# Kitware/SMQTK-Indexing

Measured on AMD Instinct MI355X. Metric: queries/sec, exact brute-force l2 kNN k=100 over 10000000x128 float32 (recall@100 = 1.0 by construction); scan HBM GB/s vs 8 TB/s peak, higher is better.
Workload: dtype f32 results (distances bit-identical to numpy float32); filter arithmetic int8 MFMA (i32 accumulation, measured per-row error bound), exact re-rank f32

## Files before the change

### smqtk_indexing_amd/csrc/sq_common.hpp

```cpp
#pragma once
#include <hip/hip_runtime.h>

#include <atomic>
#include <chrono>

#include <cstdarg>
#include <cstdint>
#include <cstdio>
#include <cstring>
#include <mutex>
#include <string>
#include <unordered_map>
#include <utility>
#include <vector>

#include "../../include/smqtk_hip.h"

typedef unsigned long long u64;
typedef unsigned int u32;

namespace sq {

extern thread_local char g_err[512];
inline int fail(int code, const char* fmt, ...) {
// ... 34 lines not shown
    int dense_qplanes = 0;
    int dense_no_center = 0;
    int dense_rerank_segments = 0;
    int merge_threads = 0;
    int spin_wait_us = 2000;
    int dense_async_streams = 2;
    int dense_async_depth = 2;
    int dense_async_wait = 1;
    int dense_async_order = 1;
    int dense_nt = -1;
    int dense_nt_keep_mb = 0;
    int hamming_no_permute = 0;
    int dense_fused_prep = 1;
    int dense_int8_batch = 64;
    int dense_fused = 1;
    int dense_tighten = 1;
    int dense_graph = 1;
    int dense_int8 = -1;
    int dense_int8_wide = 0;
    int dense_mid_tier = 1;
    int hamming_async_depth = 2;
    int hamming_async_wait = 1;
    int hamming_async_order = 1;
    int hamming_ring = -1;
    int hamming_tighten = 1;
    int hamming_fused = 1;
};
extern Options g_opt;
int Options::*option_member(const char* name);

// ... 183 lines not shown
```

### smqtk_indexing_amd/csrc/sq_core.hip

```cpp
#include <algorithm>
#include <cmath>
#include <cstdint>
#include <cstring>
#include <limits>
#include <thread>
#include <utility>
#include <vector>

#include "sq_common.hpp"

namespace sq {

thread_local char g_err[512] = "";
Options g_opt;

static std::mutex g_reg_mu;
static std::unordered_map<sq_handle_t, HandleBase*> g_reg;
static sq_handle_t g_next = 1;

sq_handle_t register_handle(HandleBase* h) {
    std::lock_guard<std::mutex> l(g_reg_mu);
    sq_handle_t id = g_next++;
    g_reg[id] = h;
    return id;
// ... 53 lines not shown
        {"sample_stride", &Options::sample_stride},
        {"candidate_cap", &Options::candidate_cap},
        {"force_fallback", &Options::force_fallback},
        {"dense_stages", &Options::dense_stages},
        {"dense_blocks", &Options::dense_blocks},
        {"dense_sample_blocks", &Options::dense_sample_blocks},
        {"dense_debug", &Options::dense_debug},
        {"dense_waves", &Options::dense_waves},
        {"dense_qt", &Options::dense_qt},
        {"itq_exact", &Options::itq_exact},
        {"hamming_no_permute", &Options::hamming_no_permute},
        {"dense_no_center", &Options::dense_no_center},
        {"merge_threads", &Options::merge_threads},
        {"spin_wait_us", &Options::spin_wait_us},
        {"dense_rerank_segments", &Options::dense_rerank_segments},
        {"dense_qplanes", &Options::dense_qplanes},
        {"dense_async_streams", &Options::dense_async_streams},
        {"dense_async_depth", &Options::dense_async_depth},
        {"dense_async_wait", &Options::dense_async_wait},
        {"dense_async_order", &Options::dense_async_order},
        {"dense_nt", &Options::dense_nt},
        {"dense_nt_keep_mb", &Options::dense_nt_keep_mb},
        {"dense_mid_tier", &Options::dense_mid_tier},
        {"dense_int8", &Options::dense_int8},
        {"dense_int8_wide", &Options::dense_int8_wide},
        {"dense_graph", &Options::dense_graph},
        {"dense_fused", &Options::dense_fused},
        {"dense_tighten", &Options::dense_tighten},
        {"dense_int8_batch", &Options::dense_int8_batch},
        {"dense_fused_prep", &Options::dense_fused_prep},
// ... 311 lines not shown
```

### smqtk_indexing_amd/csrc/sq_dense.hip

```cpp
#include <algorithm>
#include <vector>
#include <cmath>

#include "sq_dense_exact.hpp"
#include "sq_dense_scan.hpp"
#include "sq_dense_mid.hpp"
#include "sq_dense_i8.hpp"
#include "sq_dense_wide.hpp"
#include "sq_dense_i8_wide.hpp"
#include "sq_dense_tighten.hpp"
#include "sq_dense_remove.hpp"

namespace sq {

struct DenseCall {
    bool pending = false;
    const float* q = nullptr;
    int nq = 0, k = 0, nq_pad = 0;
    void* out_dist = nullptr;
    long long* out_idx = nullptr;
    hipStream_t st = nullptr;
    bool small = false, all_fallback = false, prof = false, use_event = false, int8 = false;
    bool mid_direct = false;
    u32 cap = 0;
    sq_stats_t stats{};
};
struct DenseSlot {
    DevBuf q_scaled, q_al, qn2, thr, wave_out, wave_cnt, cnt, keys, sample, out_keys, cos_nq, oflag;
    DevBuf q8, par8;
    DevBuf clk8;
    int clk8_wgs = 0;
    DevBuf wave_score, hist8;
    DevBuf tg;
    void* tg_zeroed = nullptr;
    DevBuf sort_tmp;
    HostPinned status_host;
    HostPinned call_ptrs;
// ... 252 lines not shown
template <int KS>
static int dense8_head_launch_t(const Dense8HeadArgs& a, hipStream_t st) {
    using G = I8Geom<KS>;
    constexpr int ring = G::WAVES * G::NSTAGE * G::SLOT_BYTES;
    return launch_lds<dense8_head_kernel<KS>>(ring, dim3((unsigned)a.s.nrb), dim3(G::WAVES * 64), ring, st, a);
}
static int dense8_head_launch(int row_bytes, const Dense8HeadArgs& a, hipStream_t st) {
    switch (row_bytes) {
        case 128: return dense8_head_launch_t<4>(a, st);
        case 256: return dense8_head_launch_t<8>(a, st);
        case 512: return dense8_head_launch_t<16>(a, st);
    }
    return fail(SQ_ERR_INVALID, "int8 head: unsupported row width %d", row_bytes);
}
template <int KS, bool COSINE>
static int dense8_body_launch_t(const Dense8ScanArgs& a, const Dense8TailArgs& t, hipStream_t st) {
    using G = I8Geom<KS>;
    constexpr int ring = G::WAVES * G::NSTAGE * G::SLOT_BYTES;
    return launch_lds<dense8_body_kernel<KS, COSINE>>(ring, dim3((unsigned)a.nrb), dim3(G::WAVES * 64), ring, st, a, t);
}
static int dense8_body_launch(int row_bytes, bool cosine, const Dense8ScanArgs& a, const Dense8TailArgs& t, hipStream_t st) {
    switch (row_bytes) {
        case 128: return cosine ? dense8_body_launch_t<4, true>(a, t, st) : dense8_body_launch_t<4, false>(a, t, st);
        case 256: return cosine ? dense8_body_launch_t<8, true>(a, t, st) : dense8_body_launch_t<8, false>(a, t, st);
        case 512: return cosine ? dense8_body_launch_t<16, true>(a, t, st) : dense8_body_launch_t<16, false>(a, t, st);
    }
    return fail(SQ_ERR_INVALID, "int8 body: unsupported row width %d", row_bytes);
}
static int i8_waves(int row_bytes) { return row_bytes == 512 ? I8Geom<16>::WAVES : I8Geom<4>::WAVES; }

static bool dense_mid_shape_ok(const DenseHandle* h) {
    const bool cosine = h->metric == SQ_METRIC_COSINE;
    return h->d <= 512 && (reinterpret_cast<uintptr_t>(h->db) & 15u) == 0 && (h->ld & 3) == 0 && h->ld >= (h->d + 3) / 4 * 4 && h->n >= 32 &&
           (cosine ? h->cos_nx.p != nullptr : h->norms.p != nullptr);
}

static int dense8_wide_enqueue(DenseHandle* h, DenseSlot& s, const float* q, int nq, int k, int kk, void* out_dist, long long* out_idx,
                               hipStream_t st, bool prof, u32 cap, u32* hs_dev, u32* hs_raw_dev) {
    const long long n = h->n;
    const int d = h->d, row8 = h->row8, ku = i8w_units(row8), qw = ku * I8W_UNIT;
    const bool cosine = h->metric == SQ_METRIC_COSINE;
    const size_t key_bytes = cosine ? sizeof(K128) : sizeof(u64);
// ... 310 lines not shown
            else if (per_wg <= 4.5 && keep8 > 8) keep8 = 8;
        }
        const long long lane_m = (long long)nrb_sample * keep8;
        SQ_TRY(s.sample.reserve(fused ? (size_t)TILE_ROWS * lane_m * 4 : (size_t)nq_pad * ns * 4));
        a.sample_out = s.sample.as<float>();
        if (fused) {
            SQ_TRY(s.wave_score.reserve((size_t)n_waves * wave_cap * 4));
            SQ_TRY(s.hist8.reserve((size_t)I8_HIST_WORDS * 4));
            a.wave_score = s.wave_score.as<float>();
            a.hist = s.hist8.as<u32>();
        }
        int wpb = 2;
        if (!cosine && h->opt.dense_rerank_segments > 0 && waves8 % h->opt.dense_rerank_segments == 0 && h->opt.dense_rerank_segments <= 4)
            wpb = h->opt.dense_rerank_segments;
        const size_t rr_lds = (qt == 1 && ldq <= 156) ? (size_t)32 * (ldq + 4) * 4 : 0;
        const DenseCallPtrs* ind = nullptr;
        auto chain = [&](hipStream_t cs) -> int {
            if (fused) {
                Dense8HeadArgs ha{};
                ha.s = a;
                ha.s.unit_step = stride;
                ha.s.n_sel = ns_units;
                ha.s.nrb = nrb_sample;
                ha.q = q;
                ha.nq = nq;
                ha.d = d;
                ha.center = centerp;
                ha.dx = h->dx8;
                ha.r_max = h->rmax8;
                ha.x_max = h->xmax8;
                ha.cosine = cosine ? 1 : 0;
                ha.qn2 = qn2;
                ha.cnt = cnt;
                ha.oflag = oflag;
                ha.q_al = s.q_al.as<float>();
                ha.ldq = ldq;
                ha.ind = ind;
                ha.lane_min = s.sample.as<float>();
                ha.keep = keep8;
                ha.kk = kk;
                if (const int rc = dense8_head_launch(row8, ha, cs)) return rc;
                Dense8ScanArgs b = a;
                b.unit_step = 1;
                b.n_sel = n_units;
                b.nrb = nrb;
                Dense8TailArgs ta{h->db, h->ld, d, s.q_al.as<float>(), ldq, nq, s.keys.p, cnt, cap, oflag, cnx, cnq, h->opt.dense_debug, qn2, kk, tighten ? 1 : 0, nullptr};
                s.clk8_wgs = 0;
                if ((h->opt.dense_debug & 8192) && !use_event) {
                    if (const int rc = s.clk8.reserve((size_t)nrb * 64)) return rc;
                    SQ_HIP(hipMemsetAsync(s.clk8.p, 0, (size_t)nrb * 64, cs));
                    ta.clk = s.clk8.as<long long>();
                    s.clk8_wgs = nrb;
                }
                if (prof) SQ_HIP(hipEventRecord(s.ev[1], cs));
                if (const int rc = dense8_body_launch(row8, cosine, b, ta, cs)) return rc;
                if (prof) {
                    SQ_HIP(hipEventRecord(s.ev[2], cs));
                    SQ_HIP(hipEventRecord(s.ev[4], cs));
                }
                if (cosine) {
                    DenseFinalizeCos fin{cnt, cap, kk, h->id_base, thr, 0.0, 1, (double*)out_dist, out_idx, hs_dev, hs_raw_dev, oflag, 0};
                    fin.lin = s.par8.as<float2>();
                    fin.ind = ind;
                    if (tighten) fin.thr2k = a.hist + TILE_ROWS * I8_HIST_BINS;
                    fin.cnt_shift = I8_CNT_SHIFT;
                    return select_launch_t<K128>(s.keys.as<K128>(), cnt, cap, key_stride, k, nq, s.out_keys.as<K128>(), fin, cs, s.sort_tmp, 8 * stride * kk, I8_CNT_SHIFT);
                }
                DenseFinalizeL2 fin{cnt, cap, kk, h->id_base, thr, qn2, 0.0, 1, (float*)out_dist, out_idx, hs_dev, hs_raw_dev, oflag, 0};
                fin.lin = s.par8.as<float2>();
                fin.ind = ind;
                if (tighten) fin.thr2k = a.hist + TILE_ROWS * I8_HIST_BINS;
                fin.cnt_shift = I8_CNT_SHIFT;
                return select_launch_t<u64>(s.keys.as<u64>(), cnt, cap, key_stride, k, nq, s.out_keys.as<u64>(), fin, cs, s.sort_tmp, 8 * stride * kk, I8_CNT_SHIFT);
            }
// ... 24 lines not shown
                fin.lin = s.par8.as<float2>();
                fin.ind = ind;
                return select_launch_t<K128>(s.keys.as<K128>(), cnt, cap, key_stride, k, nq, s.out_keys.as<K128>(), fin, cs, s.sort_tmp, 8 * stride * kk);
            }
            hipLaunchKernelGGL(dense_rerank_l2_kernel, dim3((unsigned)((n_waves + wpb - 1) / wpb)), dim3(128 * wpb), rr_lds, cs, h->db, h->ld, d,
                               s.q_al.as<float>(), ldq, a.wave_out, a.wave_cnt, wave_cap, n_waves, wpb, nq, group_q, s.keys.as<u64>(), cnt,
                               cap, oflag, h->opt.dense_debug);
            if (prof) SQ_HIP(hipEventRecord(s.ev[4], cs));
            DenseFinalizeL2 fin{cnt, cap, kk, h->id_base, thr, qn2, 0.0, 1, (float*)out_dist, out_idx, hs_dev, hs_raw_dev, oflag, 0};
            fin.lin = s.par8.as<float2>();
            fin.ind = ind;
            return select_launch_t<u64>(s.keys.as<u64>(), cnt, cap, key_stride, k, nq, s.out_keys.as<u64>(), fin, cs, s.sort_tmp, 8 * stride * kk);
        };
        c.stats.scan_launches = 2;
        c.stats.bytes_scanned = h->n_pad64 * ((long long)row8 + 4) * nqt;
        bool launched = false;
        if (use_event && !prof && h->opt.dense_graph != 0 && !h->graph_broken && st != nullptr && st == s.own) {
            u64 key = 0xcbf29ce484222325ull;
            auto mix = [&key](u64 v) { key = (key ^ v) * 0x100000001b3ull; };
            for (u64 v : {(u64)(fused ? 1 : 0), (u64)(tighten ? 1 : 0), (u64)(uintptr_t)s.wave_score.p, (u64)(uintptr_t)s.hist8.p, (u64)lane_m, (u64)nq, (u64)k, (u64)row8, (u64)qt, (u64)nqt, (u64)wpb, (u64)stride, (u64)nrb, (u64)nrb_sample, (u64)ns, (u64)a.nt, (u64)a.nt_from_row, (u64)n, (u64)h->n_live, (u64)cap,
                          (u64)h->opt.dense_debug, (u64)h->id_base, (u64)(uintptr_t)st, (u64)(uintptr_t)h->db, (u64)(uintptr_t)centerp,
                          (u64)(uintptr_t)h->scan8.p, (u64)(uintptr_t)h->nrow8.p, (u64)(uintptr_t)s.q8.p, (u64)(uintptr_t)s.par8.p,
                          (u64)(uintptr_t)s.sample.p, (u64)(uintptr_t)s.keys.p, (u64)(uintptr_t)s.wave_out.p, (u64)(uintptr_t)s.wave_cnt.p,
                          (u64)(uintptr_t)s.q_al.p, (u64)(uintptr_t)cnt, (u64)(uintptr_t)thr, (u64)(uintptr_t)qn2, (u64)(uintptr_t)oflag,
                          (u64)(uintptr_t)s.out_keys.p, (u64)(uintptr_t)hs_raw_dev, (u64)(uintptr_t)cnx, (u64)(uintptr_t)cnq, (u64)(cosine ? 1 : 0)})
                mix(v);
            if (key == 0) key = 1;
            if (s.gexec && s.gkey != key) {
                (void)hipGraphExecDestroy(s.gexec);
                s.gexec = nullptr;
            }
            if (!s.gexec && s.seen_key == key) {
                SQ_TRY(s.call_ptrs.reserve(sizeof(DenseCallPtrs)));
                void* ind_dev = nullptr;
                SQ_TRY(s.call_ptrs.device_ptr(&ind_dev));
// ... 223 lines not shown
    u32* cnt = s.cnt.as<u32>();
    float* thr = s.thr.as<float>();
    double* qn2 = s.qn2.as<double>();
    const double* cnx = h->cos_nx.as<double>();
    const double* cnq = s.cos_nq.as<double>();
    u32* hs_raw = reinterpret_cast<u32*>(s.status_host.p);
    u32* hs = hs_raw + c.nq_pad;
    u32* hs_raw_dev = nullptr;
    SQ_TRY(s.status_host.device_ptr(reinterpret_cast<void**>(&hs_raw_dev)));
    u32* hs_dev = hs_raw_dev + c.nq_pad;
    const size_t l2_lds = (size_t)((d + 3) / 4 * 4) * 4;
    h->stats = c.stats;
    if (!all_fallback) {
        SQ_HIP(c.use_event ? event_wait(s.ev_done) : stream_wait(st));
        SQ_HIP(hipGetLastError());
        double clk_tail_ms = -1.0;
        if (s.clk8_wgs > 0 && (h->opt.dense_debug & 8192)) {
            std::vector<long long> ck((size_t)s.clk8_wgs * 8);
            SQ_HIP(hipMemcpy(ck.data(), s.clk8.p, ck.size() * 8, hipMemcpyDeviceToHost));
            long long t0 = ck[0], tend = 0;
            for (int w = 0; w < s.clk8_wgs; ++w) t0 = std::min(t0, ck[(size_t)w * 8]), tend = std::max(tend, ck[(size_t)w * 8 + 4]);
            double sum[5] = {0, 0, 0, 0, 0}, mx[5] = {0, 0, 0, 0, 0}, mn[5] = {1e30, 1e30, 1e30, 1e30, 1e30};
            for (int w = 0; w < s.clk8_wgs; ++w) {
                const long long* e = &ck[(size_t)w * 8];
                const double v[5] = {(e[0] - t0) * 0.01, (e[1] - e[0]) * 0.01, (e[2] - e[1]) * 0.01, (e[3] - e[2]) * 0.01, (e[4] - e[3]) * 0.01};
                for (int j = 0; j < 5; ++j) sum[j] += v[j], mx[j] = std::max(mx[j], v[j]), mn[j] = std::min(mn[j], v[j]);
            }
            const char* names[5] = {"start offset", "stream (first wave out)", "wave skew (all waves out)", "thresholds", "re-rank"};
            if (h->opt.dense_debug & 16384) {
                fprintf(stderr, "[body clocks] %d workgroups, kernel span %.1f us\n", s.clk8_wgs, (tend - t0) * 0.01);
                for (int j = 0; j < 5; ++j) fprintf(stderr, "   %-28s min %8.1f  mean %8.1f  max %8.1f us\n", names[j], mn[j], sum[j] / s.clk8_wgs, mx[j]);
            }
            long long stream_end = 0;
            for (int w = 0; w < s.clk8_wgs; ++w) stream_end = std::max(stream_end, ck[(size_t)w * 8 + 2]);
            clk_tail_ms = (double)(tend - stream_end) * 1e-5;
            s.clk8_wgs = 0;
        }
        if (c.prof) {
            float t1 = 0, t2 = 0;
            SQ_HIP(hipEventElapsedTime(&t1, s.ev[1], s.ev[2]));
            SQ_HIP(hipEventElapsedTime(&t2, s.ev[0], s.ev[3]));
            h->stats.scan_ms = t1;
            h->stats.total_ms = t2;
            if (h->ev_ref) {
                float e[5] = {0, 0, 0, 0, 0};
                const int order[5] = {0, 1, 2, 4, 3};
                for (int j = 0; j < 5; ++j) (void)hipEventElapsedTime(&e[j], h->ev_ref, s.ev[order[j]]);
                fprintf(stderr, "[smqtk_hip] trace slot %d: start %.1f | head-> %.1f | scan-> %.1f | rerank-> %.1f | select-> %.1f us\n",
                        (int)(&s - h->slot), e[0] * 1e3f, e[1] * 1e3f, e[2] * 1e3f, e[3] * 1e3f, e[4] * 1e3f);
            }
            if (c.stats.scan_launches == 2) {
                float t3 = 0;
                SQ_HIP(hipEventElapsedTime(&t3, s.ev[2], s.ev[4]));
                h->stats.rerank_ms = t3;
                if (clk_tail_ms >= 0.0) h->stats.rerank_ms = clk_tail_ms;
            }
        }
        for (int qi = 0; qi < nq; ++qi) h->stats.candidates += hs_raw[qi];
        if (c.int8) {
            int over = 0;
            for (int qi = 0; qi < nq; ++qi) over += (hs[qi] & 1u) ? 1 : 0;
            long long cands = 0;
            for (int qi = 0; qi < nq; ++qi) cands += hs_raw[qi];
            const bool heavy = 2 * over > nq || cands > (long long)nq * std::max<long long>(24ll * 1024, n / 128);
            h->overflow8 = heavy ? h->overflow8 + 1 : 0;
            if (h->overflow8 >= 3 && h->opt.dense_int8 < 0) h->suspended8 = true;
        }
        if (!small && (!c.int8 || h->opt.dense_int8 > 0)) {
            int over = 0;
            for (int qi = 0; qi < nq; ++qi) over += (hs[qi] & 1u) ? 1 : 0;
// ... 1090 lines not shown
```

### smqtk_indexing_amd/csrc/sq_dense_i8.hpp

```cpp
#pragma once
#include "sq_dense_scan.hpp"

namespace sq {

typedef int i32x4 __attribute__((ext_vector_type(4)));
typedef int i32x16 __attribute__((ext_vector_type(16)));

template <int KS>
struct I8Geom {
    static constexpr int ROW_BYTES = KS * 32;
    static constexpr int UNIT_ROWS = KS == 4 ? 64 : 32;
    static constexpr int TILES = UNIT_ROWS / 32;
    static constexpr int UNIT_BYTES = UNIT_ROWS * ROW_BYTES;
    static constexpr int SLOT_BYTES = UNIT_BYTES + 256;
    static constexpr int WAVES = KS <= 8 ? 8 : 4;
    static constexpr int NSTAGE = 2;
    static constexpr int PIECES = UNIT_BYTES / 1024;
    static constexpr int SAMPLES_PER_UNIT = 2 * TILES;
};
static constexpr int I8_MAX_ROW_BYTES = 512;
__host__ __device__ constexpr int i8_row_bytes(int d) { return d <= 128 ? 128 : (d <= 256 ? 256 : 512); }
__host__ __device__ constexpr int i8_unit_rows(int row_bytes) { return row_bytes == 128 ? 64 : 32; }

__device__ __forceinline__ float i8_element(float v, const float* __restrict__ center, int k, bool cosine, double inv_norm) {
// ... 364 lines not shown
};

template <int KS>
__device__ __forceinline__ int i8_swz(int c, int r) {
    if constexpr (KS == 4) return c ^ ((r >> 1) & 7);
    return (c & ~15) | ((c & 15) ^ (r & 15));
}

enum { I8_EMIT = 0, I8_SAMPLE = 1, I8_LANEMIN = 2, I8_EMIT_H = 3 };

static constexpr int I8_HIST_BINS = 64;
static constexpr int I8_CNT_SHIFT = 5;
static constexpr int I8_HIST_WORDS = TILE_ROWS * I8_HIST_BINS + (TILE_ROWS << I8_CNT_SHIFT);

template <int WAVES>
__device__ __forceinline__ void dense8_hist_flush(u32* lds_hist, u32* __restrict__ ghist) {
    constexpr int PER = TILE_ROWS * I8_HIST_BINS / WAVES;
    const int lane = threadIdx.x & 63;
    const int wave = __builtin_amdgcn_readfirstlane(threadIdx.x >> 6);
#pragma unroll
    for (int i = 0; i < PER / 64; ++i) {
        const int b = wave * PER + i * 64 + lane;
        const u32 v = __hip_atomic_exchange(lds_hist + b, 0u, __ATOMIC_RELAXED, __HIP_MEMORY_SCOPE_WORKGROUP);
        if (v) __hip_atomic_fetch_add(ghist + b, v, __ATOMIC_RELAXED, __HIP_MEMORY_SCOPE_AGENT);
    }
}

template <int KS, int MODE>
__device__ __forceinline__ void dense8_stream(const Dense8ScanArgs& a, unsigned char* smem, const i32x4 (&bq)[KS], const i32x4 (&bl)[KS],
                                              float unit_lo, float thr_l, u32& wcount, float& smin, u32* lds_ticket,
                                              float inv_w_l = 0.f, u32* lds_hist = nullptr) {
    using G = I8Geom<KS>;
    constexpr bool SAMPLE = MODE == I8_SAMPLE || MODE == I8_LANEMIN;
    const int lane = threadIdx.x & 63;
    const int wave = __builtin_amdgcn_readfirstlane(threadIdx.x >> 6);
    const int r31 = lane & 31, h = lane >> 5;
    const u32 lds_base = (u32)(uintptr_t)smem;
    const u32 ring_base = lds_base + (u32)wave * (G::NSTAGE * G::SLOT_BYTES);
    const unsigned char* ring_ptr = smem + wave * (G::NSTAGE * G::SLOT_BYTES);
    const long long wave_id = (long long)blockIdx.x * G::WAVES + wave;
    const long long nwaves = (long long)a.nrb * G::WAVES;
    uint2* wout = a.wave_out + wave_id * a.wave_cap;
    float* wsc = MODE == I8_EMIT_H ? a.wave_score + wave_id * a.wave_cap : nullptr;
    u32* hist_l = MODE == I8_EMIT_H ? lds_hist + r31 * I8_HIST_BINS : nullptr;

    const long long wg_first = (long long)blockIdx.x * G::WAVES;
    auto take_unit = [&]() __attribute__((always_inline)) -> long long {
        u32 t = 0;
        if (lane == 0) t = __hip_atomic_fetch_add(lds_ticket, 1u, __ATOMIC_RELAXED, __HIP_MEMORY_SCOPE_WORKGROUP);
        t = (u32)__builtin_amdgcn_readfirstlane((int)t);
        const long long u = wg_first + (long long)(t % G::WAVES) + (long long)(t / G::WAVES) * nwaves;
        return u < a.n_sel ? u : -1ll;
    };
    const long long my_units = wave_id < a.n_sel ? (a.n_sel - wave_id + nwaves - 1) / nwaves : 0;
    u32 voff[G::PIECES];
#pragma unroll
    for (int j = 0; j < G::PIECES; ++j) {
        const int lin = j * 1024 + lane * 16;
        const int r = lin / G::ROW_BYTES, cpos = (lin % G::ROW_BYTES) >> 4;
        voff[j] = (u32)(r * G::ROW_BYTES + i8_swz<KS>(cpos, r) * 16);
    }
    const u32 voff_n = (u32)lane * 4u;
    static_assert(G::NSTAGE == 2, "two ring slots: the units in flight are sel_even / sel_odd");
    long long issued = 0, sel_even = -1, sel_odd = -1;
    bool more = true;
    auto issue_next = [&]() __attribute__((always_inline)) {
        if (!more) return;
        const long long sel = take_unit();
        if (sel < 0) {
// ... 4 lines not shown
        const long long unit_idx = sel * a.unit_step;
        const long long row0 = unit_idx * G::UNIT_ROWS;
        const u32 dst = ring_base + (u32)(issued % G::NSTAGE) * G::SLOT_BYTES;
        const unsigned char* base = reinterpret_cast<const unsigned char*>(a.scan8) + row0 * G::ROW_BYTES;
#pragma unroll
        for (int j = 0; j < G::PIECES; ++j) {
            if (a.nt && row0 >= a.nt_from_row)
                glds16<true>(base, voff[j], dst + (u32)j * 1024);
            else
                glds16<false>(base, voff[j], dst + (u32)j * 1024);
        }
        glds4(a.nrow + row0, voff_n, dst + G::UNIT_BYTES);
        ++issued;
    };
    for (int p = 0; p < G::NSTAGE; ++p) issue_next();
    const int flush_every = (int)(my_units >> 3) > 0 ? (int)(my_units >> 3) : 1;
    int to_flush = flush_every;

    for (long long it = 0; it < issued; ++it) {
        const long long sel = (it & 1) ? sel_odd : sel_even;
        const long long unit_idx = sel * a.unit_step;
        const long long row0 = unit_idx * G::UNIT_ROWS;
        wait_units_in_flight<G::NSTAGE, G::PIECES + 1>((int)(issued - it - 1));
        const unsigned char* sl = ring_ptr + (it % G::NSTAGE) * G::SLOT_BYTES;
        constexpr int KH = KS == 16 ? 8 : KS;
        i32x4 av[G::TILES][KH];
        f32x4 nr[G::TILES][4];
#pragma unroll
        for (int t = 0; t < G::TILES; ++t) {
            const int r = 32 * t + r31;
#pragma unroll
            for (int s = 0; s < KH; ++s)
                av[t][s] = *reinterpret_cast<const i32x4*>(sl + r * G::ROW_BYTES + i8_swz<KS>(2 * s + h, r) * 16);
// ... 52 lines not shown
                    if (mask) {
                        const u32 pos = wcount + __builtin_amdgcn_mbcnt_hi((u32)(bal >> 32), __builtin_amdgcn_mbcnt_lo((u32)bal, 0u));
                        if (pos < a.wave_cap) {
                            wout[pos] = make_uint2((u32)(row0 + 32 * t + 4 * h), (mask << 16) | (u32)r31);
                            if constexpr (MODE == I8_EMIT_H) wsc[pos] = m;
                        }
                        if constexpr (MODE == I8_EMIT_H) {
                            if (m > -__builtin_inff()) {
                                const int bin = min((int)((thr_l - m) * inv_w_l), I8_HIST_BINS - 1);
                                __hip_atomic_fetch_add(hist_l + bin, 1u, __ATOMIC_RELAXED, __HIP_MEMORY_SCOPE_WORKGROUP);
                            }
                        }
                    }
                    wcount += (u32)__popcll(bal);
                }
            }
        }
        if constexpr (MODE == I8_EMIT_H) {
            if (--to_flush == 0) {
                to_flush = flush_every;
                dense8_hist_flush<G::WAVES>(lds_hist, a.hist);
            }
        }
    }
}

template <int KS>
__device__ __forceinline__ void dense8_load_planes(const signed char* planes, i32x4 (&bq)[KS], i32x4 (&bl)[KS]) {
    using G = I8Geom<KS>;
    const int lane = threadIdx.x & 63, r31 = lane & 31, h = lane >> 5;
#pragma unroll
    for (int s = 0; s < KS; ++s) {
        bq[s] = *reinterpret_cast<const i32x4*>(planes + r31 * G::ROW_BYTES + (2 * s + h) * 16);
        bl[s] = *reinterpret_cast<const i32x4*>(planes + (TILE_ROWS + r31) * G::ROW_BYTES + (2 * s + h) * 16);
    }
#pragma unroll
// ... 223 lines not shown
    const float* db;
    long long ld;
    int d;
    const float* q_al;
    int ldq, nq;
    void* keys;
    u32* cnt;
    u32 cap;
    u32* overflow;
    const double* nx64;
    const double* nq64;
    int debug;
    const double* qn2;
    int kk;
    int tighten;
    long long* clk;
};
static constexpr int I8_TAIL_QROWS_BYTES = 32 * (156 + 4) * 4;
static constexpr int I8_TAIL_LIST = 2048;
static constexpr int I8_TAIL_RERANK_BYTES = I8_TAIL_QROWS_BYTES + 3 * RERANK_MAX_GROUP * 4 + 8 * 32 * RERANK_STAGE_STRIDE * 4;
static constexpr int I8_TAIL_LDS_BYTES = I8_TAIL_RERANK_BYTES + I8_TAIL_LIST * 8 + TILE_ROWS * 4 + 16;

template <int KS, bool COSINE>
__global__ __launch_bounds__(I8Geom<KS>::WAVES * 64, KS == 16 ? 1 : 2) void dense8_body_kernel(Dense8ScanArgs a, Dense8TailArgs ta) {
    using G = I8Geom<KS>;
    static_assert(I8_TAIL_LDS_BYTES <= G::WAVES * G::NSTAGE * G::SLOT_BYTES, "the re-rank works in the ring's LDS");
    extern __shared__ __attribute__((aligned(16))) unsigned char smem[];
    __shared__ u32 s_hist8[TILE_ROWS * I8_HIST_BINS];
    __shared__ u32 s_wcnt[G::WAVES];
    __shared__ u32 s_unit_ticket;
    __shared__ float s_thr1[TILE_ROWS], s_eq[TILE_ROWS];
    __shared__ double s_qn2b[TILE_ROWS];
    __shared__ float2 s_parb[TILE_ROWS];
    if (threadIdx.x == 0) s_unit_ticket = 0u;
    if (threadIdx.x < TILE_ROWS) {
        s_thr1[threadIdx.x] = a.thr[threadIdx.x];
        s_parb[threadIdx.x] = a.par[threadIdx.x];
        s_eq[threadIdx.x] = a.par[threadIdx.x].y;
        s_qn2b[threadIdx.x] = ta.qn2[threadIdx.x];
    }
    const int lane = threadIdx.x & 63;
    const int wave = __builtin_amdgcn_readfirstlane(threadIdx.x >> 6);
    const int r31 = lane & 31;
    for (int i = threadIdx.x; i < TILE_ROWS * I8_HIST_BINS; i += G::WAVES * 64) s_hist8[i] = 0u;
    long long* clk = ta.clk ? ta.clk + (long long)blockIdx.x * 8 : nullptr;
    if (clk && threadIdx.x == 0) {
        clk[0] = (long long)wall_clock64();
        clk[1] = 0x7fffffffffffffffll;
    }
    __syncthreads();
    i32x4 bq[KS], bl[KS];
    dense8_load_planes<KS>(a.qs8, bq, bl);
    float unit_lo = a.par[r31].x * 0.00390625f;
    float thr_l = a.thr[r31];
    const float eq_l = a.par[r31].y;
    float inv_w_l = (eq_l > 0.f && eq_l < __builtin_inff()) ? 2.f / eq_l : 0.f;
    if (!(inv_w_l < 3.0e38f)) inv_w_l = 0.f;
    asm volatile("" : "+v"(unit_lo), "+v"(thr_l), "+v"(inv_w_l));
    u32 wcount = 0;
    float smin = 0.f;
    dense8_stream<KS, I8_EMIT_H>(a, smem, bq, bl, unit_lo, thr_l, wcount, smin, &s_unit_ticket, inv_w_l, s_hist8);
    const long long w0 = (long long)blockIdx.x * G::WAVES;
    if (lane == 0) {
        a.wave_cnt[2 * (w0 + wave)] = wcount;
        a.wave_cnt[2 * (w0 + wave) + 1] = 0u;
        s_wcnt[wave] = wcount;
        if (clk) atomicMin((unsigned long long*)(clk + 1), (unsigned long long)wall_clock64());
    }
    asm volatile("s_waitcnt vmcnt(0) lgkmcnt(0)" ::: "memory");
    __builtin_amdgcn_fence(__ATOMIC_RELEASE, "workgroup");
    __syncthreads();
    __builtin_amdgcn_fence(__ATOMIC_ACQUIRE, "workgroup");
    if (clk && threadIdx.x == 0) clk[2] = (long long)wall_clock64();
    float* fl = reinterpret_cast<float*>(smem);
    u32* su = reinterpret_cast<u32*>(smem + I8_TAIL_QROWS_BYTES);
    RerankLds L{fl, su, su + RERANK_MAX_GROUP, su + 2 * RERANK_MAX_GROUP,
                COSINE ? reinterpret_cast<float*>(smem + I8_TAIL_QROWS_BYTES + 3 * RERANK_MAX_GROUP * 4) : nullptr};
    {
        uint2* s_list = reinterpret_cast<uint2*>(smem + I8_TAIL_RERANK_BYTES);
        float* s_thr2 = reinterpret_cast<float*>(smem + I8_TAIL_RERANK_BYTES + I8_TAIL_LIST * 8);
        u32* s_npass = reinterpret_cast<u32*>(s_thr2 + TILE_ROWS);
        static_assert(I8_HIST_BINS == 64, "one lane per bin");
        bool any = false;
#pragma unroll
        for (int wi = 0; wi < G::WAVES; ++wi) any = any || s_wcnt[wi] != 0u;
        const Dense8ThrPost post{s_parb, s_qn2b};
        constexpr int NQW = TILE_ROWS / G::WAVES;
        u32 hc[NQW];
        if (ta.tighten && any) {
#pragma unroll
            for (int j = 0; j < NQW; ++j) {
                const int qi = (j >> 2) * 4 * G::WAVES + wave * 4 + (j & 3);
                hc[j] = __hip_atomic_load(a.hist + qi * I8_HIST_BINS + lane, __ATOMIC_RELAXED, __HIP_MEMORY_SCOPE_AGENT);
            }
#pragma unroll
            for (int j = 0; j < NQW; ++j) {
                const int qi = (j >> 2) * 4 * G::WAVES + wave * 4 + (j & 3);
                hc[j] += s_hist8[qi * I8_HIST_BINS + lane];
            }
        }
#pragma unroll
        for (int rnd = 0; rnd < TILE_ROWS / (4 * G::WAVES); ++rnd) {
#pragma unroll
            for (int j = 0; j < 4; ++j) {
                const int qi = rnd * 4 * G::WAVES + wave * 4 + j;
                const float t1 = s_thr1[qi];
                float t2 = t1;
                if (ta.tighten && any && qi < ta.nq && t1 < __builtin_inff() && t1 > -__builtin_inff()) {
                    u32 c = hc[rnd * 4 + j];
#pragma unroll
                    for (int o = 1; o < 64; o <<= 1) {
                        const u32 up = (u32)__shfl_down((int)c, o);
                        c += lane + o < 64 ? up : 0u;
                    }
                    const u64 reach = __ballot(c >= (u32)ta.kk);
                    const float eq = s_eq[qi];
                    if (reach != 0ull && eq > 0.f && eq < __builtin_inff()) {
                        const int jb = 63 - __clzll((long long)reach);
                        const float inv_w = 2.f / eq;
                        if (inv_w < 3.0e38f) {
                            const double t8 = (double)t1 - (double)jb / (double)inv_w * (1.0 - 1e-6);
                            float t8f = (float)t8;
                            if ((double)t8f < t8) t8f = __uint_as_float(__float_as_uint(t8f) + (t8f >= 0.f ? 1 : -1));
                            const float cand = post(qi, t8f);
                            if (cand < t2) t2 = cand;
                        }
                    }
                    if (lane == 0) atomicMax(a.hist + TILE_ROWS * I8_HIST_BINS + (qi << I8_CNT_SHIFT), ordered_f32(t2));
                }
                if (lane == 0) s_thr2[qi] = t2;
            }
        }
        if (ta.tighten) {
            L.scores = a.wave_score;
            L.thr2 = s_thr2;
            L.list = s_list;
            L.npass = s_npass;
            L.list_cap = I8_TAIL_LIST;
        }
        L.seg_cnt = s_wcnt;
        L.cnt_shift = I8_CNT_SHIFT;
        __syncthreads();
        if (clk && threadIdx.x == 0) clk[3] = (long long)wall_clock64();
        if (ta.tighten) dense8_hist_flush<G::WAVES>(s_hist8, a.hist);
    }
    using K = typename std::conditional<COSINE, K128, u64>::type;
    rerank_block<K, COSINE>(ta.db, ta.ld, ta.d, ta.q_al, ta.ldq, ta.nq, TILE_ROWS, a.wave_out, a.wave_cnt, a.wave_cap,
                            (long long)a.nrb * G::WAVES, G::WAVES, static_cast<K*>(ta.keys), ta.cnt, ta.cap, ta.overflow, ta.nx64,
                            ta.nq64, ta.debug, w0, L);
    if (clk) {
        asm volatile("s_waitcnt vmcnt(0) lgkmcnt(0)" ::: "memory");
        __syncthreads();
        if (threadIdx.x == 0) clk[4] = (long long)wall_clock64();
    }
}

template <int QT, bool SAMPLE>
__global__ __launch_bounds__(512, 2) void dense8_scan_mt_kernel(Dense8ScanArgs a) {
    using G = I8Geom<4>;
    extern __shared__ __attribute__((aligned(16))) unsigned char smem[];
    const int lane = threadIdx.x & 63;
    const int wave = __builtin_amdgcn_readfirstlane(threadIdx.x >> 6);
    const int r31 = lane & 31, h = lane >> 5;
    const u32 lds_base = (u32)(uintptr_t)smem;
    const u32 ring_base = lds_base + (u32)wave * (G::NSTAGE * G::SLOT_BYTES);
    const unsigned char* ring_ptr = smem + wave * (G::NSTAGE * G::SLOT_BYTES);
    const long long wave_id = (long long)blockIdx.x * G::WAVES + wave;
    uint2* wout = a.wave_out + wave_id * a.wave_cap;
// ... 124 lines not shown
```

Before: 144,000.

## Split fused int8 body kernel into separate scan and tail re-rank kernels

```diff
diff --git a/smqtk_indexing_amd/csrc/sq_common.hpp b/smqtk_indexing_amd/csrc/sq_common.hpp
--- a/smqtk_indexing_amd/csrc/sq_common.hpp
+++ b/smqtk_indexing_amd/csrc/sq_common.hpp
@@ -72,6 +72,7 @@
     int dense_fused_prep = 1;
     int dense_int8_batch = 64;
     int dense_fused = 1;
+    int dense_tail_blocks = 0;
     int dense_tighten = 1;
     int dense_graph = 1;
     int dense_int8 = -1;
diff --git a/smqtk_indexing_amd/csrc/sq_core.hip b/smqtk_indexing_amd/csrc/sq_core.hip
--- a/smqtk_indexing_amd/csrc/sq_core.hip
+++ b/smqtk_indexing_amd/csrc/sq_core.hip
@@ -91,6 +91,7 @@
         {"merge_threads", &Options::merge_threads},
         {"spin_wait_us", &Options::spin_wait_us},
         {"dense_rerank_segments", &Options::dense_rerank_segments},
+        {"dense_tail_blocks", &Options::dense_tail_blocks},
         {"dense_qplanes", &Options::dense_qplanes},
         {"dense_async_streams", &Options::dense_async_streams},
         {"dense_async_depth", &Options::dense_async_depth},
diff --git a/smqtk_indexing_amd/csrc/sq_dense.hip b/smqtk_indexing_amd/csrc/sq_dense.hip
--- a/smqtk_indexing_amd/csrc/sq_dense.hip
+++ b/smqtk_indexing_amd/csrc/sq_dense.hip
@@ -21,6 +21,7 @@
     long long* out_idx = nullptr;
     hipStream_t st = nullptr;
     bool small = false, all_fallback = false, prof = false, use_event = false, int8 = false;
+    bool tail_in_scan = false;
     bool mid_direct = false;
     u32 cap = 0;
     sq_stats_t stats{};
@@ -303,18 +304,22 @@
     return fail(SQ_ERR_INVALID, "int8 head: unsupported row width %d", row_bytes);
 }
 template <int KS, bool COSINE>
-static int dense8_body_launch_t(const Dense8ScanArgs& a, const Dense8TailArgs& t, hipStream_t st) {
+static int dense8_body_launch_t(const Dense8ScanArgs& a, long long* clk, hipStream_t st) {
     using G = I8Geom<KS>;
     constexpr int ring = G::WAVES * G::NSTAGE * G::SLOT_BYTES;
-    return launch_lds<dense8_body_kernel<KS, COSINE>>(ring, dim3((unsigned)a.nrb), dim3(G::WAVES * 64), ring, st, a, t);
-}
-static int dense8_body_launch(int row_bytes, bool cosine, const Dense8ScanArgs& a, const Dense8TailArgs& t, hipStream_t st) {
+    return launch_lds<dense8_body_kernel<KS, COSINE>>(ring, dim3((unsigned)a.nrb), dim3(G::WAVES * 64), ring, st, a, clk);
+}
+static int dense8_body_launch(int row_bytes, bool cosine, const Dense8ScanArgs& a, long long* clk, hipStream_t st) {
     switch (row_bytes) {
-        case 128: return cosine ? dense8_body_launch_t<4, true>(a, t, st) : dense8_body_launch_t<4, false>(a, t, st);
-        case 256: return cosine ? dense8_body_launch_t<8, true>(a, t, st) : dense8_body_launch_t<8, false>(a, t, st);
-        case 512: return cosine ? dense8_body_launch_t<16, true>(a, t, st) : dense8_body_launch_t<16, false>(a, t, st);
+        case 128: return cosine ? dense8_body_launch_t<4, true>(a, clk, st) : dense8_body_launch_t<4, false>(a, clk, st);
+        case 256: return cosine ? dense8_body_launch_t<8, true>(a, clk, st) : dense8_body_launch_t<8, false>(a, clk, st);
+        case 512: return cosine ? dense8_body_launch_t<16, true>(a, clk, st) : dense8_body_launch_t<16, false>(a, clk, st);
     }
     return fail(SQ_ERR_INVALID, "int8 body: unsupported row width %d", row_bytes);
+}
+static int dense8_tail_launch(bool cosine, int blocks, size_t lds, const Dense8TailArgs& t, hipStream_t st) {
+    return cosine ? launch<dense8_tail_kernel<true>>(dim3((unsigned)blocks), dim3(I8_TAIL_WAVES * 64), lds, st, t)
+                  : launch<dense8_tail_kernel<false>>(dim3((unsigned)blocks), dim3(I8_TAIL_WAVES * 64), lds, st, t);
 }
 static int i8_waves(int row_bytes) { return row_bytes == 512 ? I8Geom<16>::WAVES : I8Geom<4>::WAVES; }
 
@@ -655,6 +660,7 @@
         if (!cosine && h->opt.dense_rerank_segments > 0 && waves8 % h->opt.dense_rerank_segments == 0 && h->opt.dense_rerank_segments <= 4)
             wpb = h->opt.dense_rerank_segments;
         const size_t rr_lds = (qt == 1 && ldq <= 156) ? (size_t)32 * (ldq + 4) * 4 : 0;
+        const int tail_blocks = h->opt.dense_tail_blocks > 0 ? h->opt.dense_tail_blocks : nrb;
         const DenseCallPtrs* ind = nullptr;
         auto chain = [&](hipStream_t cs) -> int {
             if (fused) {
@@ -685,20 +691,45 @@
                 b.unit_step = 1;
                 b.n_sel = n_units;
                 b.nrb = nrb;
-                Dense8TailArgs ta{h->db, h->ld, d, s.q_al.as<float>(), ldq, nq, s.keys.p, cnt, cap, oflag, cnx, cnq, h->opt.dense_debug, qn2, kk, tighten ? 1 : 0, nullptr};
+                long long* clk = nullptr;
                 s.clk8_wgs = 0;
                 if ((h->opt.dense_debug & 8192) && !use_event) {
                     if (const int rc = s.clk8.reserve((size_t)nrb * 64)) return rc;
                     SQ_HIP(hipMemsetAsync(s.clk8.p, 0, (size_t)nrb * 64, cs));
-                    ta.clk = s.clk8.as<long long>();
+                    clk = s.clk8.as<long long>();
                     s.clk8_wgs = nrb;
                 }
                 if (prof) SQ_HIP(hipEventRecord(s.ev[1], cs));
-                if (const int rc = dense8_body_launch(row8, cosine, b, ta, cs)) return rc;
-                if (prof) {
-                    SQ_HIP(hipEventRecord(s.ev[2], cs));
-                    SQ_HIP(hipEventRecord(s.ev[4], cs));
-                }
+                if (const int rc = dense8_body_launch(row8, cosine, b, clk, cs)) return rc;
+                if (prof) SQ_HIP(hipEventRecord(s.ev[2], cs));
+                Dense8TailArgs ta{};
+                ta.db = h->db;
+                ta.ld = h->ld;
+                ta.d = d;
+                ta.q_al = s.q_al.as<float>();
+                ta.ldq = ldq;
+                ta.nq = nq;
+                ta.keys = s.keys.p;
+                ta.cnt = cnt;
+                ta.cap = cap;
+                ta.overflow = oflag;
+                ta.nx64 = cnx;
+                ta.nq64 = cnq;
+                ta.debug = h->opt.dense_debug;
+                ta.qn2 = qn2;
+                ta.kk = kk;
+                ta.tighten = tighten ? 1 : 0;
+                ta.par = a.par;
+                ta.thr = thr;
+                ta.wave_out = a.wave_out;
+                ta.wave_score = a.wave_score;
+                ta.wave_cnt = a.wave_cnt;
+                ta.wave_cap = wave_cap;
+                ta.n_waves = n_waves;
+                ta.segs = waves8;
+                ta.hist = a.hist;
+                if (const int rc = dense8_tail_launch(cosine, std::min(tail_blocks, nrb), rr_lds, ta, cs)) return rc;
+                if (prof) SQ_HIP(hipEventRecord(s.ev[4], cs));
                 if (cosine) {
                     DenseFinalizeCos fin{cnt, cap, kk, h->id_base, thr, 0.0, 1, (double*)out_dist, out_idx, hs_dev, hs_raw_dev, oflag, 0};
                     fin.lin = s.par8.as<float2>();
@@ -753,11 +784,12 @@
         };
         c.stats.scan_launches = 2;
         c.stats.bytes_scanned = h->n_pad64 * ((long long)row8 + 4) * nqt;
+        c.tail_in_scan = fused;
         bool launched = false;
         if (use_event && !prof && h->opt.dense_graph != 0 && !h->graph_broken && st != nullptr && st == s.own) {
             u64 key = 0xcbf29ce484222325ull;
             auto mix = [&key](u64 v) { key = (key ^ v) * 0x100000001b3ull; };
-            for (u64 v : {(u64)(fused ? 1 : 0), (u64)(tighten ? 1 : 0), (u64)(uintptr_t)s.wave_score.p, (u64)(uintptr_t)s.hist8.p, (u64)lane_m, (u64)nq, (u64)k, (u64)row8, (u64)qt, (u64)nqt, (u64)wpb, (u64)stride, (u64)nrb, (u64)nrb_sample, (u64)ns, (u64)a.nt, (u64)a.nt_from_row, (u64)n, (u64)h->n_live, (u64)cap,
+            for (u64 v : {(u64)(fused ? 1 : 0), (u64)(tighten ? 1 : 0), (u64)tail_blocks, (u64)(uintptr_t)s.wave_score.p, (u64)(uintptr_t)s.hist8.p, (u64)lane_m, (u64)nq, (u64)k, (u64)row8, (u64)qt, (u64)nqt, (u64)wpb, (u64)stride, (u64)nrb, (u64)nrb_sample, (u64)ns, (u64)a.nt, (u64)a.nt_from_row, (u64)n, (u64)h->n_live, (u64)cap,
                           (u64)h->opt.dense_debug, (u64)h->id_base, (u64)(uintptr_t)st, (u64)(uintptr_t)h->db, (u64)(uintptr_t)centerp,
                           (u64)(uintptr_t)h->scan8.p, (u64)(uintptr_t)h->nrow8.p, (u64)(uintptr_t)s.q8.p, (u64)(uintptr_t)s.par8.p,
                           (u64)(uintptr_t)s.sample.p, (u64)(uintptr_t)s.keys.p, (u64)(uintptr_t)s.wave_out.p, (u64)(uintptr_t)s.wave_cnt.p,
@@ -1011,31 +1043,27 @@
     if (!all_fallback) {
         SQ_HIP(c.use_event ? event_wait(s.ev_done) : stream_wait(st));
         SQ_HIP(hipGetLastError());
-        double clk_tail_ms = -1.0;
         if (s.clk8_wgs > 0 && (h->opt.dense_debug & 8192)) {
             std::vector<long long> ck((size_t)s.clk8_wgs * 8);
             SQ_HIP(hipMemcpy(ck.data(), s.clk8.p, ck.size() * 8, hipMemcpyDeviceToHost));
             long long t0 = ck[0], tend = 0;
-            for (int w = 0; w < s.clk8_wgs; ++w) t0 = std::min(t0, ck[(size_t)w * 8]), tend = std::max(tend, ck[(size_t)w * 8 + 4]);
-            double sum[5] = {0, 0, 0, 0, 0}, mx[5] = {0, 0, 0, 0, 0}, mn[5] = {1e30, 1e30, 1e30, 1e30, 1e30};
+            for (int w = 0; w < s.clk8_wgs; ++w) t0 = std::min(t0, ck[(size_t)w * 8]), tend = std::max(tend, ck[(size_t)w * 8 + 2]);
+            double sum[3] = {0, 0, 0}, mx[3] = {0, 0, 0}, mn[3] = {1e30, 1e30, 1e30};
             for (int w = 0; w < s.clk8_wgs; ++w) {
                 const long long* e = &ck[(size_t)w * 8];
-                const double v[5] = {(e[0] - t0) * 0.01, (e[1] - e[0]) * 0.01, (e[2] - e[1]) * 0.01, (e[3] - e[2]) * 0.01, (e[4] - e[3]) * 0.01};
-                for (int j = 0; j < 5; ++j) sum[j] += v[j], mx[j] = std::max(mx[j], v[j]), mn[j] = std::min(mn[j], v[j]);
-            }
-            const char* names[5] = {"start offset", "stream (first wave out)", "wave skew (all waves out)", "thresholds", "re-rank"};
+                const double v[3] = {(e[0] - t0) * 0.01, (e[1] - e[0]) * 0.01, (e[2] - e[1]) * 0.01};
+                for (int j = 0; j < 3; ++j) sum[j] += v[j], mx[j] = std::max(mx[j], v[j]), mn[j] = std::min(mn[j], v[j]);
+            }
+            const char* names[3] = {"start offset", "stream (first wave out)", "wave skew (all waves out)"};
             if (h->opt.dense_debug & 16384) {
-                fprintf(stderr, "[body clocks] %d workgroups, kernel span %.1f us\n", s.clk8_wgs, (tend - t0) * 0.01);
-                for (int j = 0; j < 5; ++j) fprintf(stderr, "   %-28s min %8.1f  mean %8.1f  max %8.1f us\n", names[j], mn[j], sum[j] / s.clk8_wgs, mx[j]);
-            }
-            long long stream_end = 0;
-            for (int w = 0; w < s.clk8_wgs; ++w) stream_end = std::max(stream_end, ck[(size_t)w * 8 + 2]);
-            clk_tail_ms = (double)(tend - stream_end) * 1e-5;
+                fprintf(stderr, "[body clocks] %d workgroups, span to the last wave out %.1f us\n", s.clk8_wgs, (tend - t0) * 0.01);
+                for (int j = 0; j < 3; ++j) fprintf(stderr, "   %-28s min %8.1f  mean %8.1f  max %8.1f us\n", names[j], mn[j], sum[j] / s.clk8_wgs, mx[j]);
+            }
             s.clk8_wgs = 0;
         }
         if (c.prof) {
             float t1 = 0, t2 = 0;
-            SQ_HIP(hipEventElapsedTime(&t1, s.ev[1], s.ev[2]));
+            SQ_HIP(hipEventElapsedTime(&t1, s.ev[1], s.ev[c.tail_in_scan ? 4 : 2]));
             SQ_HIP(hipEventElapsedTime(&t2, s.ev[0], s.ev[3]));
             h->stats.scan_ms = t1;
             h->stats.total_ms = t2;
@@ -1050,7 +1078,6 @@
                 float t3 = 0;
                 SQ_HIP(hipEventElapsedTime(&t3, s.ev[2], s.ev[4]));
                 h->stats.rerank_ms = t3;
-                if (clk_tail_ms >= 0.0) h->stats.rerank_ms = clk_tail_ms;
             }
         }
         for (int qi = 0; qi < nq; ++qi) h->stats.candidates += hs_raw[qi];
diff --git a/smqtk_indexing_amd/csrc/sq_dense_i8.hpp b/smqtk_indexing_amd/csrc/sq_dense_i8.hpp
--- a/smqtk_indexing_amd/csrc/sq_dense_i8.hpp
+++ b/smqtk_indexing_amd/csrc/sq_dense_i8.hpp
@@ -402,14 +402,14 @@
 static constexpr int I8_HIST_WORDS = TILE_ROWS * I8_HIST_BINS + (TILE_ROWS << I8_CNT_SHIFT);
 
 template <int WAVES>
-__device__ __forceinline__ void dense8_hist_flush(u32* lds_hist, u32* __restrict__ ghist) {
+__device__ __forceinline__ void dense8_hist_flush(const u32* lds_hist, u32* __restrict__ ghist) {
     constexpr int PER = TILE_ROWS * I8_HIST_BINS / WAVES;
     const int lane = threadIdx.x & 63;
     const int wave = __builtin_amdgcn_readfirstlane(threadIdx.x >> 6);
 #pragma unroll
     for (int i = 0; i < PER / 64; ++i) {
         const int b = wave * PER + i * 64 + lane;
-        const u32 v = __hip_atomic_exchange(lds_hist + b, 0u, __ATOMIC_RELAXED, __HIP_MEMORY_SCOPE_WORKGROUP);
+        const u32 v = lds_hist[b];
         if (v) __hip_atomic_fetch_add(ghist + b, v, __ATOMIC_RELAXED, __HIP_MEMORY_SCOPE_AGENT);
     }
 }
@@ -440,7 +440,6 @@
         const long long u = wg_first + (long long)(t % G::WAVES) + (long long)(t / G::WAVES) * nwaves;
         return u < a.n_sel ? u : -1ll;
     };
-    const long long my_units = wave_id < a.n_sel ? (a.n_sel - wave_id + nwaves - 1) / nwaves : 0;
     u32 voff[G::PIECES];
 #pragma unroll
     for (int j = 0; j < G::PIECES; ++j) {
@@ -475,9 +474,6 @@
         ++issued;
     };
     for (int p = 0; p < G::NSTAGE; ++p) issue_next();
-    const int flush_every = (int)(my_units >> 3) > 0 ? (int)(my_units >> 3) : 1;
-    int to_flush = flush_every;
-
     for (long long it = 0; it < issued; ++it) {
         const long long sel = (it & 1) ? sel_odd : sel_even;
         const long long unit_idx = sel * a.unit_step;
@@ -560,12 +556,6 @@
                     }
                     wcount += (u32)__popcll(bal);
                 }
-            }
-        }
-        if constexpr (MODE == I8_EMIT_H) {
-            if (--to_flush == 0) {
-                to_flush = flush_every;
-                dense8_hist_flush<G::WAVES>(lds_hist, a.hist);
             }
         }
     }
@@ -819,36 +809,31 @@
     const double* qn2;
     int kk;
     int tighten;
-    long long* clk;
+    const float2* par;
+    const float* thr;
+    const uint2* wave_out;
+    const float* wave_score;
+    const u32* wave_cnt;
+    u32 wave_cap;
+    long long n_waves;
+    int segs;
+    u32* hist;
 };
-static constexpr int I8_TAIL_QROWS_BYTES = 32 * (156 + 4) * 4;
+static constexpr int I8_TAIL_WAVES = 4;
 static constexpr int I8_TAIL_LIST = 2048;
-static constexpr int I8_TAIL_RERANK_BYTES = I8_TAIL_QROWS_BYTES + 3 * RERANK_MAX_GROUP * 4 + 8 * 32 * RERANK_STAGE_STRIDE * 4;
-static constexpr int I8_TAIL_LDS_BYTES = I8_TAIL_RERANK_BYTES + I8_TAIL_LIST * 8 + TILE_ROWS * 4 + 16;
 
 template <int KS, bool COSINE>
-__global__ __launch_bounds__(I8Geom<KS>::WAVES * 64, KS == 16 ? 1 : 2) void dense8_body_kernel(Dense8ScanArgs a, Dense8TailArgs ta) {
+__global__ __launch_bounds__(I8Geom<KS>::WAVES * 64, KS == 16 ? 1 : 2) void dense8_body_kernel(Dense8ScanArgs a, long long* clk_all) {
     using G = I8Geom<KS>;
-    static_assert(I8_TAIL_LDS_BYTES <= G::WAVES * G::NSTAGE * G::SLOT_BYTES, "the re-rank works in the ring's LDS");
     extern __shared__ __attribute__((aligned(16))) unsigned char smem[];
     __shared__ u32 s_hist8[TILE_ROWS * I8_HIST_BINS];
-    __shared__ u32 s_wcnt[G::WAVES];
     __shared__ u32 s_unit_ticket;
-    __shared__ float s_thr1[TILE_ROWS], s_eq[TILE_ROWS];
-    __shared__ double s_qn2b[TILE_ROWS];
-    __shared__ float2 s_parb[TILE_ROWS];
     if (threadIdx.x == 0) s_unit_ticket = 0u;
-    if (threadIdx.x < TILE_ROWS) {
-        s_thr1[threadIdx.x] = a.thr[threadIdx.x];
-        s_parb[threadIdx.x] = a.par[threadIdx.x];
-        s_eq[threadIdx.x] = a.par[threadIdx.x].y;
-        s_qn2b[threadIdx.x] = ta.qn2[threadIdx.x];
-    }
     const int lane = threadIdx.x & 63;
     const int wave = __builtin_amdgcn_readfirstlane(threadIdx.x >> 6);
     const int r31 = lane & 31;
     for (int i = threadIdx.x; i < TILE_ROWS * I8_HIST_BINS; i += G::WAVES * 64) s_hist8[i] = 0u;
-    long long* clk = ta.clk ? ta.clk + (long long)blockIdx.x * 8 : nullptr;
+    long long* clk = clk_all ? clk_all + (long long)blockIdx.x * 8 : nullptr;
     if (clk && threadIdx.x == 0) {
         clk[0] = (long long)wall_clock64();
         clk[1] = 0x7fffffffffffffffll;
@@ -869,94 +854,90 @@
     if (lane == 0) {
         a.wave_cnt[2 * (w0 + wave)] = wcount;
         a.wave_cnt[2 * (w0 + wave) + 1] = 0u;
-        s_wcnt[wave] = wcount;
         if (clk) atomicMin((unsigned long long*)(clk + 1), (unsigned long long)wall_clock64());
     }
-    asm volatile("s_waitcnt vmcnt(0) lgkmcnt(0)" ::: "memory");
-    __builtin_amdgcn_fence(__ATOMIC_RELEASE, "workgroup");
+    asm volatile("s_waitcnt lgkmcnt(0)" ::: "memory");
     __syncthreads();
-    __builtin_amdgcn_fence(__ATOMIC_ACQUIRE, "workgroup");
     if (clk && threadIdx.x == 0) clk[2] = (long long)wall_clock64();
-    float* fl = reinterpret_cast<float*>(smem);
-    u32* su = reinterpret_cast<u32*>(smem + I8_TAIL_QROWS_BYTES);
-    RerankLds L{fl, su, su + RERANK_MAX_GROUP, su + 2 * RERANK_MAX_GROUP,
-                COSINE ? reinterpret_cast<float*>(smem + I8_TAIL_QROWS_BYTES + 3 * RERANK_MAX_GROUP * 4) : nullptr};
-    {
-        uint2* s_list = reinterpret_cast<uint2*>(smem + I8_TAIL_RERANK_BYTES);
-        float* s_thr2 = reinterpret_cast<float*>(smem + I8_TAIL_RERANK_BYTES + I8_TAIL_LIST * 8);
-        u32* s_npass = reinterpret_cast<u32*>(s_thr2 + TILE_ROWS);
-        static_assert(I8_HIST_BINS == 64, "one lane per bin");
-        bool any = false;
-#pragma unroll
-        for (int wi = 0; wi < G::WAVES; ++wi) any = any || s_wcnt[wi] != 0u;
-        const Dense8ThrPost post{s_parb, s_qn2b};
-        constexpr int NQW = TILE_ROWS / G::WAVES;
-        u32 hc[NQW];
-        if (ta.tighten && any) {
-#pragma unroll
-            for (int j = 0; j < NQW; ++j) {
-                const int qi = (j >> 2) * 4 * G::WAVES + wave * 4 + (j & 3);
-                hc[j] = __hip_atomic_load(a.hist + qi * I8_HIST_BINS + lane, __ATOMIC_RELAXED, __HIP_MEMORY_SCOPE_AGENT);
-            }
-#pragma unroll
-            for (int j = 0; j < NQW; ++j) {
-                const int qi = (j >> 2) * 4 * G::WAVES + wave * 4 + (j & 3);
-                hc[j] += s_hist8[qi * I8_HIST_BINS + lane];
-            }
-        }
-#pragma unroll
-        for (int rnd = 0; rnd < TILE_ROWS / (4 * G::WAVES); ++rnd) {
-#pragma unroll
-            for (int j = 0; j < 4; ++j) {
-                const int qi = rnd * 4 * G::WAVES + wave * 4 + j;
-                const float t1 = s_thr1[qi];
-                float t2 = t1;
-                if (ta.tighten && any && qi < ta.nq && t1 < __builtin_inff() && t1 > -__builtin_inff()) {
-                    u32 c = hc[rnd * 4 + j];
-#pragma unroll
-                    for (int o = 1; o < 64; o <<= 1) {
-                        const u32 up = (u32)__shfl_down((int)c, o);
-                        c += lane + o < 64 ? up : 0u;
+    dense8_hist_flush<G::WAVES>(s_hist8, a.hist);
+}
+
+template <bool COSINE>
+__global__ __launch_bounds__(I8_TAIL_WAVES * 64) void dense8_tail_kernel(Dense8TailArgs ta) {
+    extern __shared__ __attribute__((aligned(16))) float s_qrows_dyn[];
+    __shared__ u32 s_hist[RERANK_MAX_GROUP], s_base[RERANK_MAX_GROUP], s_fill[RERANK_MAX_GROUP];
+    __shared__ __attribute__((aligned(16))) float s_stage[COSINE ? I8_TAIL_WAVES : 1][COSINE ? 32 * RERANK_STAGE_STRIDE : 1];
+    __shared__ uint2 s_list[I8_TAIL_LIST];
+    __shared__ float s_thr1[TILE_ROWS], s_eq[TILE_ROWS], s_thr2[TILE_ROWS];
+    __shared__ double s_qn2b[TILE_ROWS];
+    __shared__ float2 s_parb[TILE_ROWS];
+    __shared__ u32 s_npass;
+    static_assert(I8_HIST_BINS == 64, "one lane per bin");
+    const int lane = threadIdx.x & 63;
+    const int wave = __builtin_amdgcn_readfirstlane(threadIdx.x >> 6);
+    if (threadIdx.x < TILE_ROWS) {
+        s_thr1[threadIdx.x] = ta.thr[threadIdx.x];
+        s_parb[threadIdx.x] = ta.par[threadIdx.x];
+        s_eq[threadIdx.x] = ta.par[threadIdx.x].y;
+        s_qn2b[threadIdx.x] = ta.qn2[threadIdx.x];
+    }
+    constexpr int NQW = TILE_ROWS / I8_TAIL_WAVES;
+    u32 hc[NQW] = {};
+    if (ta.tighten) {
+#pragma unroll
+        for (int j = 0; j < NQW; ++j) {
+            const int qi = (j >> 2) * 4 * I8_TAIL_WAVES + wave * 4 + (j & 3);
+            hc[j] = ta.hist[qi * I8_HIST_BINS + lane];
+        }
+    }
+    __syncthreads();
+    const Dense8ThrPost post{s_parb, s_qn2b};
+#pragma unroll
+    for (int rnd = 0; rnd < TILE_ROWS / (4 * I8_TAIL_WAVES); ++rnd) {
+#pragma unroll
+        for (int j = 0; j < 4; ++j) {
+            const int qi = rnd * 4 * I8_TAIL_WAVES + wave * 4 + j;
+            const float t1 = s_thr1[qi];
+            float t2 = t1;
+            if (ta.tighten && qi < ta.nq && t1 < __builtin_inff() && t1 > -__builtin_inff()) {
+                u32 c = hc[rnd * 4 + j];
+#pragma unroll
+                for (int o = 1; o < 64; o <<= 1) {
+                    const u32 up = (u32)__shfl_down((int)c, o);
+                    c += lane + o < 64 ? up : 0u;
+                }
+                const u64 reach = __ballot(c >= (u32)ta.kk);
+                const float eq = s_eq[qi];
+                if (reach != 0ull && eq > 0.f && eq < __builtin_inff()) {
+                    const int jb = 63 - __clzll((long long)reach);
+                    const float inv_w = 2.f / eq;
+                    if (inv_w < 3.0e38f) {
+                        const double t8 = (double)t1 - (double)jb / (double)inv_w * (1.0 - 1e-6);
+                        float t8f = (float)t8;
+                        if ((double)t8f < t8) t8f = __uint_as_float(__float_as_uint(t8f) + (t8f >= 0.f ? 1 : -1));
+                        const float cand = post(qi, t8f);
+                        if (cand < t2) t2 = cand;
                     }
-                    const u64 reach = __ballot(c >= (u32)ta.kk);
-                    const float eq = s_eq[qi];
-                    if (reach != 0ull && eq > 0.f && eq < __builtin_inff()) {
-                        const int jb = 63 - __clzll((long long)reach);
-                        const float inv_w = 2.f / eq;
-                        if (inv_w < 3.0e38f) {
-                            const double t8 = (double)t1 - (double)jb / (double)inv_w * (1.0 - 1e-6);
-                            float t8f = (float)t8;
-                            if ((double)t8f < t8) t8f = __uint_as_float(__float_as_uint(t8f) + (t8f >= 0.f ? 1 : -1));
-                            const float cand = post(qi, t8f);
-                            if (cand < t2) t2 = cand;
-                        }
-                    }
-                    if (lane == 0) atomicMax(a.hist + TILE_ROWS * I8_HIST_BINS + (qi << I8_CNT_SHIFT), ordered_f32(t2));
                 }
-                if (lane == 0) s_thr2[qi] = t2;
-            }
-        }
-        if (ta.tighten) {
-            L.scores = a.wave_score;
-            L.thr2 = s_thr2;
-            L.list = s_list;
-            L.npass = s_npass;
-            L.list_cap = I8_TAIL_LIST;
-        }
-        L.seg_cnt = s_wcnt;
-        L.cnt_shift = I8_CNT_SHIFT;
+                if (lane == 0 && blockIdx.x == 0) ta.hist[TILE_ROWS * I8_HIST_BINS + (qi << I8_CNT_SHIFT)] = ordered_f32(t2);
+            }
+            if (lane == 0) s_thr2[qi] = t2;
+        }
+    }
+    RerankLds L{s_qrows_dyn, s_hist, s_base, s_fill, COSINE ? &s_stage[0][0] : nullptr};
+    if (ta.tighten) {
+        L.scores = ta.wave_score;
+        L.thr2 = s_thr2;
+        L.list = s_list;
+        L.npass = &s_npass;
+        L.list_cap = I8_TAIL_LIST;
+    }
+    L.cnt_shift = I8_CNT_SHIFT;
+    using K = typename std::conditional<COSINE, K128, u64>::type;
+    for (long long w0 = (long long)blockIdx.x * ta.segs; w0 < ta.n_waves; w0 += (long long)gridDim.x * ta.segs) {
         __syncthreads();
-        if (clk && threadIdx.x == 0) clk[3] = (long long)wall_clock64();
-        if (ta.tighten) dense8_hist_flush<G::WAVES>(s_hist8, a.hist);
-    }
-    using K = typename std::conditional<COSINE, K128, u64>::type;
-    rerank_block<K, COSINE>(ta.db, ta.ld, ta.d, ta.q_al, ta.ldq, ta.nq, TILE_ROWS, a.wave_out, a.wave_cnt, a.wave_cap,
-                            (long long)a.nrb * G::WAVES, G::WAVES, static_cast<K*>(ta.keys), ta.cnt, ta.cap, ta.overflow, ta.nx64,
-                            ta.nq64, ta.debug, w0, L);
-    if (clk) {
-        asm volatile("s_waitcnt vmcnt(0) lgkmcnt(0)" ::: "memory");
-        __syncthreads();
-        if (threadIdx.x == 0) clk[4] = (long long)wall_clock64();
+        rerank_block<K, COSINE>(ta.db, ta.ld, ta.d, ta.q_al, ta.ldq, ta.nq, TILE_ROWS, ta.wave_out, ta.wave_cnt, ta.wave_cap, ta.n_waves,
+                                ta.segs, static_cast<K*>(ta.keys), ta.cnt, ta.cap, ta.overflow, ta.nx64, ta.nq64, ta.debug, w0, L);
     }
 }
 
```

Result: faster. 146,900, median of 6 (+2.0%).
